# tensorlayer/TLXCV

Hardware: AMD Instinct MI355X
Metric: images/sec fwd (higher is better)
Workload: dtype f16; 1 GPU; ResNet-50 fp16 forward, 224x224, batch 256 per GPU (BASELINE configs[1]); global_batch=256, per_gpu_batch=256, weights=seeded random (tlxcv_amd.seeded, seed 1), parallelism=single GPU, launch=hipGraph replay of the forward

## Files before the change

include/tlxmi.h:

```cpp
#ifndef TLXMI_H
#define TLXMI_H

#include <stddef.h>
#include <stdint.h>

#ifdef __cplusplus
extern "C" {
#endif

#define TLXMI_VERSION 101

typedef enum tlxmi_status {
    TLXMI_OK = 0,
    TLXMI_ERR_BAD_ARG = -1,
    TLXMI_ERR_UNSUPPORTED = -2,
    TLXMI_ERR_ALIGNMENT = -3,
    TLXMI_ERR_LAUNCH = -4,
    TLXMI_ERR_NO_DEVICE = -5
} tlxmi_status;

typedef enum tlxmi_dtype { TLXMI_F16 = 0, TLXMI_F32 = 1 } tlxmi_dtype;

typedef enum tlxmi_act {
    TLXMI_ACT_NONE = 0,
// ... 89 lines not shown
typedef struct tlxmi_seam_desc {
    int32_t dtype;
    int64_t rows;
    int32_t K1, N1, N2;
    int32_t t2_ld, skip_ld, y_ld, t1_ld;
    int32_t act;
} tlxmi_seam_desc;
int tlxmi_bottleneck_seam_supported(int dtype, int K1, int N1, int N2);
int tlxmi_bottleneck_seam_proj(const tlxmi_seam_desc* d, const void* t2, const void* w3_packed, const float* scale3,
                               const float* shift3, const void* x, const void* wd_packed, const float* scale_d,
                               const float* shift_d, void* y, const void* w1_packed, const float* scale1,
                               const float* shift1, void* t1, void* stream);
int tlxmi_bottleneck_seam(const tlxmi_seam_desc* d, const void* t2, const void* w3_packed, const float* scale3,
                          const float* shift3, const void* skip, void* y, const void* w1_packed, const float* scale1,
                          const float* shift1, void* t1, void* stream);

int tlxmi_group_conv_chunks(int Cin, int Cout, int groups, int dtype);
size_t tlxmi_packed_group_filter_bytes(int Cout, int Cin, int R, int S, int groups, int dtype);
int tlxmi_pack_group_filter(const float* src_oihw, void* dst, int Cout, int Cin, int R, int S, int groups,
                            int dtype, void* stream);
int tlxmi_group_conv2d(const tlxmi_conv2d_desc* d, int groups, const void* x, const void* w_packed,
                       const float* scale, const float* shift, const void* res, void* y, void* stream);
int tlxmi_group_conv2d_small_supported(const tlxmi_conv2d_desc* d, int groups);

int tlxmi_linear_splitk(int dtype, int64_t rows, int K, int Cout, int x_ld, const void* x, const void* w_packed,
                        int splits, void* partials, const float* scale, const float* shift, const void* res,
                        int res_ld, int act, float act_param, uint32_t flags, void* y, int y_ld, void* stream);

int tlxmi_conv2d_splitk_supported(const tlxmi_conv2d_desc* d, int splits);
int tlxmi_conv2d_splitk(const tlxmi_conv2d_desc* d, int splits, const void* x, const void* w_packed, void* partials,
// ... 176 lines not shown
```

tlxcv_amd/_lib.py:

```python
import ctypes as C
import os

_HERE = os.path.dirname(os.path.abspath(__file__))
LIB_PATH = os.path.join(_HERE, "libtlxmi.so")

F16, F32 = 0, 1
ACT_NONE, ACT_RELU, ACT_RELU6, ACT_LEAKY, ACT_HARDSWISH, ACT_HARDSIGMOID, ACT_GELU, ACT_SIGMOID, ACT_SILU = range(9)
EPI_RES_AFTER_ACT = 1
EPI_MAXPOOL_3S2P1 = 4
PLAN_SHARED_HALF = 0x100
PLAN_SHARED_FULL = 0x200
LAYOUT_NHWC, LAYOUT_NCHW = 0, 1


class ConvDesc(C.Structure):
    _fields_ = [(n, C.c_int32) for n in (
        "dtype", "N", "H", "W", "C", "Cout", "R", "S", "stride_h", "stride_w", "pad_h", "pad_w",
        "dil_h", "dil_w", "Ho", "Wo", "x_ld", "y_ld", "res_ld", "y_nstride", "res_nstride", "act")] + [
        ("act_param", C.c_float), ("flags", C.c_uint32)]


class DwConvDesc(C.Structure):
    _fields_ = [(n, C.c_int32) for n in (
        "dtype", "N", "H", "W", "C", "R", "S", "stride_h", "stride_w", "pad_h", "pad_w", "dil_h",
# ... 29 lines not shown
        ("scale", C.c_float), ("mask_mode", C.c_int32)] + [(n, C.c_int64) for n in (
            "q_batch_stride", "q_row_stride", "k_batch_stride", "k_row_stride", "v_batch_stride", "v_row_stride",
            "out_batch_stride", "out_row_stride")]


class CswinAttnDesc(C.Structure):
    _fields_ = [(n, C.c_int32) for n in ("dtype", "B", "H", "W", "hd")] + [("scale", C.c_float)] + [
        (n, C.c_int32) for n in ("branches", "heads")] + [("hs", C.c_int32 * 2), ("ws", C.c_int32 * 2)] + [(n, C.c_int64) for n in (
            "q_batch_stride", "q_row_stride", "k_batch_stride", "k_row_stride", "v_batch_stride", "v_row_stride",
            "out_batch_stride", "out_row_stride")]


class SeamDesc(C.Structure):
    _fields_ = [("dtype", C.c_int32), ("rows", C.c_int64)] + [(n, C.c_int32) for n in (
        "K1", "N1", "N2", "t2_ld", "skip_ld", "y_ld", "t1_ld", "act")]


class PreprocDesc(C.Structure):
    _fields_ = [(n, C.c_int32) for n in ("N", "H", "W", "C", "out_h", "out_w", "kh", "kw", "out_dtype", "layout", "fold_b",
                                         "cpad", "normalize")]


_vp, _i, _f, _u, _l = C.c_void_p, C.c_int, C.c_float, C.c_uint32, C.c_int64

PROTOTYPES = {
    "tlxmi_nchw_to_nhwc": [_vp, _i, _vp, _i, _i, _i, _i, _i, _i, _vp],
    "tlxmi_nchw_to_nhwc_s2d": [_vp, _i, _vp, _i, _i, _i, _i, _i, _i, _i, _vp],
    "tlxmi_patchify": [_vp, _i, _vp, _i, _i, _i, _i, _i, _i, _i, _vp],
    "tlxmi_patch_embed4": [_vp, _i, _vp, _vp, _vp, _vp, _vp, _i, _i, _i, _i, _f, _vp],
    "tlxmi_patch_embed4_pos": [_vp, _i, _vp, _vp, _vp, _vp, _vp, _vp, _i, _i, _i, _i, _f, _vp],
    "tlxmi_nhwc_to_nchw": [_vp, _i, _i, _vp, _i, _i, _i, _i, _i, _vp],
    "tlxmi_pack_filter": [_vp, _vp, _i, _i, _i, _i, _i, _vp],
    "tlxmi_fold_bn": [_vp, _vp, _vp, _vp, _vp, _f, _i, _vp, _vp, _vp],
    "tlxmi_conv2d": [C.POINTER(ConvDesc), _vp, _vp, _vp, _vp, _vp, _vp, _vp],
    "tlxmi_conv2d_splitk": [C.POINTER(ConvDesc), _i, _vp, _vp, _vp, _vp, _vp, _vp, _vp, _vp],
    "tlxmi_bottleneck_seam": [C.POINTER(SeamDesc), _vp, _vp, _vp, _vp, _vp, _vp, _vp, _vp, _vp, _vp, _vp],
    "tlxmi_bottleneck_seam_proj": [C.POINTER(SeamDesc), _vp, _vp, _vp, _vp, _vp, _vp, _vp, _vp, _vp, _vp, _vp, _vp, _vp, _vp],
    "tlxmi_preprocess_u8": [C.POINTER(PreprocDesc), _vp, _vp, _vp, _vp, _vp, _vp, _vp, _vp, _vp, _vp],
    "tlxmi_preprocess_linear_u8": [C.POINTER(PreprocDesc), _vp, _vp, _vp, _vp, _vp, _vp, _vp, _vp, _vp],
    "tlxmi_yolo_iou_aware": [_vp, _vp, _i, _l, _i, _i, _f, _vp],
    "tlxmi_yolo_box": [_vp, _i, _i, _i, _i, _i, _i, _i, _vp, _vp, _f, _i, _i, _f, _vp, _vp, _i, _i, _vp],
    "tlxmi_multiclass_nms": [_vp, _vp, _i, _i, _i, _f, _f, _i, _vp, _vp, _vp, _vp],
    "tlxmi_multiclass_nms_index": [_vp, _vp, _i, _i, _i, _f, _f, _i, _vp, _vp, _vp, _vp, _vp],
    "tlxmi_linear_splitk": [_i, _l, _i, _i, _i, _vp, _vp, _i, _vp, _vp, _vp, _vp, _i, _i, _f, _u, _vp, _i, _vp],
    "tlxmi_group_conv2d": [C.POINTER(ConvDesc), _i, _vp, _vp, _vp, _vp, _vp, _vp, _vp],
    "tlxmi_pack_group_filter": [_vp, _vp, _i, _i, _i, _i, _i, _i, _vp],
    "tlxmi_dwconv2d": [C.POINTER(DwConvDesc), _vp, _vp, _vp, _vp, _vp, _vp],
    "tlxmi_maxpool2d": [_vp, _vp, _i, _i, _i, _i, _i, _i, _i, _i, _i, _i, _i, _i, _i, _i, _i, _vp],
    "tlxmi_avgpool2d": [_vp, _vp, _i, _i, _i, _i, _i, _i, _i, _i, _i, _i, _i, _i, _i, _i, _i, _vp],
    "tlxmi_radix_gap": [_vp, _vp, _i, _i, _i, _i, _i, _i, _i, _vp],
    "tlxmi_split_attention": [_vp, _vp, _vp, _vp, _i, _i, _i, _i, _i, _i, _i, _i, _i, _vp],
    "tlxmi_global_avgpool": [_vp, _vp, _i, _i, _i, _i, _i, _i, _vp],
# ... 30 lines not shown
    "tlxmi_mul": [_vp, _vp, _vp, _i, _l, _i, _i, _i, _i, _vp],
}
_SPECIAL = {
    "tlxmi_version": ([], C.c_int),
    "tlxmi_last_error": ([], C.c_char_p),
    "tlxmi_device_count": ([], C.c_int),
    "tlxmi_packed_filter_bytes": ([_i, _i, _i, _i, _i], C.c_size_t),
    "tlxmi_packed_group_filter_bytes": ([_i, _i, _i, _i, _i, _i], C.c_size_t),
    "tlxmi_group_conv_chunks": ([_i, _i, _i, _i], C.c_int),
    "tlxmi_group_conv2d_small_supported": ([C.POINTER(ConvDesc), _i], C.c_int),
    "tlxmi_conv2d_maxpool_supported": ([C.POINTER(ConvDesc)], C.c_int),
    "tlxmi_conv2d_splitk_supported": ([C.POINTER(ConvDesc), _i], C.c_int),
    "tlxmi_preprocess_u8_workspace_bytes": ([C.POINTER(PreprocDesc)], C.c_size_t),
    "tlxmi_multiclass_nms_workspace_bytes": ([_i, _i], C.c_size_t),
    "tlxmi_bottleneck_seam_supported": ([_i, _i, _i, _i], C.c_int),
    "tlxmi_linear_ln_supported": ([_i, _l, _i, _i, _i, _i], C.c_int),
    "tlxmi_mlp_seam_supported": ([_i, _i, _i, _i], C.c_int),
    "tlxmi_sepconv2d_supported": ([C.POINTER(SepConvDesc)], C.c_int),
    "tlxmi_dwconv7_stats_supported": ([C.POINTER(DwConv7Desc)], C.c_int),
    "tlxmi_preact_conv1x1_supported": ([_i, _l, _i, _i, _i, _i, _i, _i], C.c_int),
    "tlxmi_sr_attention_supported": ([C.POINTER(MhaDesc)], C.c_int),
    "tlxmi_cswin_attention_supported": ([C.POINTER(CswinAttnDesc)], C.c_int),
    "tlxmi_lka_dw_supported": ([C.POINTER(LkaDwDesc)], C.c_int),
    "tlxmi_lka_gate_supported": ([C.POINTER(LkaGateDesc)], C.c_int),
}
ALL_SYMBOLS = sorted(list(PROTOTYPES) + list(_SPECIAL))

TUNE_LIB_PATH = os.environ.get("TLXMI_TUNE_LIB") or os.path.join(_HERE, "libtlxmi_tune.so")

_lib = None
# ... 67 lines not shown
```

tlxcv_amd/csrc/conv_igemm.hip:

```cpp
#include "common.h"
#include <stdio.h>
#include "gemm256.h"
#include "conv_halo.h"
#include "group_conv.h"
#include <stdlib.h>
#include <string.h>

namespace tlxmi {

struct ConvArgs {
    const char* x;
    const char* w;
    char* y;
    const float* scale;
    const float* shift;
    const char* res;
    int N, H, W, C, Cout, R, S, sh, sw, ph, pw, dh, dw, Ho, Wo;
    int x_ld, y_ld, res_ld;
    long y_nstride, res_nstride;
    int strided_n;
    int out_f32;
    int pp_slices;
    int act;
    float act_param;
// ... 474 lines not shown
    if (lds > 64 * 1024)
        if (int rc = raise_lds_limit(fn, 160 * 1024, "conv2d")) return rc;
    void* args[] = {&b};
    hipError_t e = hipLaunchKernel(fn, dim3((unsigned)grid, (unsigned)a.nchunk), dim3(WGM * 128), args, lds, st);
    if (e != hipSuccess) return fail(TLXMI_ERR_LAUNCH, "conv2d: HIP launch failed: %s", hipGetErrorString(e));
    return TLXMI_OK;
}

static bool pp_conv_offsets_ok(int W, int R, int S, int ph, int pw, int dh, int dw, int x_ld, int es) {
    const long long px = (long long)x_ld * es;
    const long long lead = ((long long)ph * W + pw) * px;
    const long long reach = ((long long)(R - 1) * dh * W + (long long)(S - 1) * dw + 1) * px;
    return lead < (1ll << 30) && reach < (1ll << 30);
}

template <typename T> static int dispatch(const ConvArgs& a, hipStream_t st, bool allow_stream = true, bool allow_split = true) {
    const bool pool = (a.flags & TLXMI_EPI_MAXPOOL_3S2P1) != 0;
    if constexpr (sizeof(T) == 2) {
        const int PB = a.C * 2;
        if (pool) {
            if (!(a.nchunk == 1 && !a.overhang && a.sh == 1 && a.sw == 1 && a.dh == 1 && a.dw == 1 && conv_halo_pool_ok(a.R, a.S, PB, a.Ho, a.Wo) &&
                  conv_halo_pool_act_ok(a.act) && !a.strided_n && a.vec_io && !a.res && a.Cout % 8 == 0 && a.Cout <= 128 && a.y_bytes != 0))
                return fail(TLXMI_ERR_UNSUPPORTED, "conv2d: TLXMI_EPI_MAXPOOL_3S2P1 needs the fp16 4x4 / 16-channel stem geometry (Wo = 112, even Ho, no residual)");
            HaloArgs h;
            h.x = a.x; h.w = a.w; h.y = a.y; h.scale = a.scale; h.shift = a.shift; h.res = nullptr;
            h.N = a.N; h.H = a.H; h.W = a.W; h.Cout = a.Cout; h.R = a.R; h.S = a.S; h.ph = a.ph; h.pw = a.pw;
            h.Ho = a.Ho; h.Wo = a.Wo; h.HoWo = a.HoWo; h.x_ld = a.x_ld; h.y_ld = a.y_ld; h.res_ld = 0;
            h.PB = PB; h.Kp_bytes = a.Kp_bytes; h.act = a.act; h.act_param = a.act_param; h.flags = a.flags;
            h.tpi = a.Ho / 2;
            h.ntn = (a.Cout + 63) / 64; h.nt = 0;
// ... 30 lines not shown
            h.x_bytes = a.x_bytes; h.w_bytes = a.w_bytes; h.y_bytes = a.y_bytes;
            h.res_bytes = a.res ? (unsigned)((long long)a.M * a.res_ld * 2) : 0u;
            if ((long)h.nring * h.PWp * PB + 512 <= 160 * 1024) {
                trace_launched("halo", a.M, a.Cout);
                return launch_conv_halo(h, st, num_cus());
            }
        }
    }
    if (pool) return fail(TLXMI_ERR_UNSUPPORTED, "conv2d: TLXMI_EPI_MAXPOOL_3S2P1 is an fp16-only fusion");
    struct Cand { int bm, bn; float eff; };
    const double flops = 2.0 * a.M * (double)a.Cout * a.kchunks * (16 / (int)sizeof(T));
    const double obytes = (double)a.M * a.Cout * sizeof(T) * (a.res ? 2.0 : 1.0);
    const double obi = obytes / flops;
    constexpr int NC = 12;
    Cand cands[NC] = {{128, 128, 1.00f}, {64, 128, 0.85f}, {128, 64, 0.85f}, {64, 64, 0.70f}, {256, 128, 0.90f},
                      {256, 256, 1.12f}, {256, 128, 1.20f}, {256, 256, 1.40f}, {256, 256, 1.50f}, {128, 256, 1.25f},
                      {256, 128, 1.25f}, {256, 256, 0.f}};
    const bool gemm128_ok = a.nchunk == 1 && a.R == 1 && a.S == 1 && a.ph == 0 && a.pw == 0 && a.sh == 1 && a.sw == 1 && !a.strided_n &&
                            a.vec_io && a.Cout % 8 == 0 && a.y_bytes != 0 && a.Cout >= 128 && a.ktiles >= 2 &&
                            (!a.res || (long long)a.M * a.res_ld * (long long)sizeof(T) < (1ll << 31));
    const bool gemm256_ok = gemm128_ok && a.Cout >= 256;
    const int tpk = a.cpt / 8;
    const bool strided1x1 = a.R == 1 && a.S == 1 && a.ph == 0 && a.pw == 0 && (a.sh > 1 || a.sw > 1);
    const bool as_conv = !(a.R == 1 && a.S == 1 && a.ph == 0 && a.pw == 0 && a.sh == 1 && a.sw == 1);
    const bool dilated = a.dh != 1 || a.dw != 1;
    const bool pp_dil_ok = !dilated || (tune_int("TLXMI_PP_DIL", 1) != 0 && pp_conv_offsets_ok(a.W, a.R, a.S, a.ph, a.pw, a.dh, a.dw, a.x_ld, (int)sizeof(T)));
    const bool pp_conv128_ok = a.nchunk == 1 && !a.overhang && ((a.S == 3 && a.R <= 3) || strided1x1) && pp_dil_ok && !a.strided_n &&
                               a.vec_io && a.Cout % 8 == 0 && a.Cout >= 128 && a.y_bytes != 0 && a.cpt % 8 == 0 && (tpk & (tpk - 1)) == 0 &&
                               (!a.res || (long long)a.M * a.res_ld * (long long)sizeof(T) < (1ll << 31));
    const bool pp_conv_ok = pp_conv128_ok && a.Cout >= 256;
    const long wreg = tune_int("TLXMI_WREG", 1);
// ... 572 lines not shown
    d.x_ld = x_ld; d.y_ld = Cout; d.act = TLXMI_ACT_NONE;
    const int rc = conv2d_impl(&d, splits, x, w_packed, nullptr, nullptr, nullptr, partials, stream, false, true, pstride * 4);
    if (rc != TLXMI_OK) return rc;
    const long total = (long)rows * Cout;
    const unsigned grid = (unsigned)((total + 255) / 256 < 8192 ? (total + 255) / 256 : 8192);
    if (dtype == TLXMI_F16)
        hipLaunchKernelGGL((splitk_reduce_kernel<half_t>), dim3(grid), dim3(256), 0, as_stream(stream), (const float*)partials, splits, (long)rows, Cout,
                           (long)pstride, scale, shift, (const half_t*)res, res_ld, act, act_param, flags, (half_t*)y, y_ld);
    else
        hipLaunchKernelGGL((splitk_reduce_kernel<float>), dim3(grid), dim3(256), 0, as_stream(stream), (const float*)partials, splits, (long)rows, Cout,
                           (long)pstride, scale, shift, (const float*)res, res_ld, act, act_param, flags, (float*)y, y_ld);
    return check_launch("linear_splitk");
}

namespace tlxmi {
static inline int cin_pad(int Cin, int dtype) { const int v = 16 / (int)elt_size(dtype); return (Cin + v - 1) / v * v; }
static inline int kpad_elems(int Cin, int R, int S, int dtype);
static int kpad_elems_of(int Cin, int R, int S, int dtype) { return kpad_elems(Cin, R, S, dtype); }
static inline int kpad_elems(int Cin, int R, int S, int dtype) {
    const int es = (int)elt_size(dtype);
    const int kbytes = R * S * cin_pad(Cin, dtype) * es;
    return ((kbytes + 127) / 128 * 128) / es;
}
template <typename T>
__global__ void pack_filter_kernel(const float* __restrict__ src, T* __restrict__ dst, int Cout, int Cin, int R,
                                   int S, int Cinp, int Kp, long total) {
    for (long i = (long)blockIdx.x * blockDim.x + threadIdx.x; i < total; i += (long)gridDim.x * blockDim.x) {
        const int k = (int)(i % Kp);
        const int o = (int)(i / Kp);
        const int c = k % Cinp, tap = k / Cinp;
// ... 68 lines not shown
```

tlxcv_amd/csrc/gemm256.h:

```cpp
#pragma once
#include <hip/hip_runtime.h>

namespace tlxmi {

struct Gemm256Args {
    const char* x;
    const char* w;
    char* y;
    const float* scale;
    const float* shift;
    const char* res;
    const float* rowstats = nullptr;
    float* stats_out = nullptr;
    int ln_planes = 0;
    float ln_inv_c = 0.f, ln_eps = 0.f;
    int M, Cout, x_ld, y_ld, res_ld;
    int kchunks;
    int ksteps;
    int Kp_bytes;
    int act;
    float act_param;
    unsigned flags;
    int mtiles, ntiles;
    int tiles_full = 0, tiles_total = 0, m_full = 0;
    int gn;
    unsigned x_bytes, w_bytes, y_bytes, res_bytes;
    int debug;
    int conv;
    int cH, cW, cWo, cHoWo, csh, csw, cph, cpw;
    int ctshift, ctaps;
    int kslices = 1, kt_slice = 0;
    long long slice_bytes = 0;
    int cdh = 1, cdw = 1;
};

int launch_gemm256(int dtype, int variant, const Gemm256Args& a, hipStream_t st);
int launch_gemm_pp(int dtype, const Gemm256Args& a, hipStream_t st);
int launch_gemm_pp128(int dtype, const Gemm256Args& a, hipStream_t st);
int launch_gemm_pp_n128(int dtype, const Gemm256Args& a, hipStream_t st);
bool gemm_stream_ok(int dtype, const Gemm256Args& a);
int launch_gemm_stream(int dtype, const Gemm256Args& a, hipStream_t st, int cus);

bool gemm_w4_ok(int dtype, const Gemm256Args& a);
int launch_gemm_w4(int dtype, const Gemm256Args& a, hipStream_t st, int cus);

bool gemm_wreg_ok(int dtype, const Gemm256Args& a);
int launch_gemm_wreg(const Gemm256Args& a, hipStream_t st);

}
```

tlxcv_amd/csrc/gemm_pp.hip:

```cpp
#include "common.h"
#include "gemm256.h"
#include <stdlib.h>

namespace tlxmi {

typedef __attribute__((address_space(3))) void* lds_ptr_pp_t;
static __device__ __forceinline__ void pp_dma16(__amdgpu_buffer_rsrc_t rsrc, char* lds, int voff) {
    __builtin_amdgcn_raw_ptr_buffer_load_lds(rsrc, (lds_ptr_pp_t)lds, 16, voff, 0, 0, 0);
}
static __device__ __forceinline__ __amdgpu_buffer_rsrc_t pp_srd(const char* p, unsigned bytes) {
    return __builtin_amdgcn_make_buffer_rsrc(const_cast<char*>(p), 0, bytes, 0x00020000);
}
static __device__ __forceinline__ u32x4 pp_load16(__amdgpu_buffer_rsrc_t rsrc, int voff) {
    return __builtin_amdgcn_raw_buffer_load_b128(rsrc, voff, 0, 0);
}
static __device__ __forceinline__ void pp_store16_nt(__amdgpu_buffer_rsrc_t rsrc, u32x4 v, int voff) {
    __builtin_amdgcn_raw_buffer_store_b128(v, rsrc, voff, 0, 2);
}
static __device__ __forceinline__ void pp_store16_wb(__amdgpu_buffer_rsrc_t rsrc, u32x4 v, int voff) {
    __builtin_amdgcn_raw_buffer_store_b128(v, rsrc, voff, 0, 0);
}

template <typename T> struct MmaPP;
template <> struct MmaPP<half_t> {
    static __device__ __forceinline__ f32x4 run(u32x4 a, u32x4 b, f32x4 c) {
        return __builtin_amdgcn_mfma_f32_16x16x32_f16(__builtin_bit_cast(half8v, a), __builtin_bit_cast(half8v, b), c, 0, 0, 0);
    }
};
template <> struct MmaPP<float> {
    static __device__ __forceinline__ f32x4 run(u32x4 a, u32x4 b, f32x4 c) {
        f32x4 af = __builtin_bit_cast(f32x4, a), bf = __builtin_bit_cast(f32x4, b);
#pragma unroll
        for (int j = 0; j < 4; ++j) c = __builtin_amdgcn_mfma_f32_16x16x4f32(af[j], bf[j], c, 0, 0, 0);
        return c;
    }
};

template <typename T, int HM, int HN, bool CONV, bool LNF = false, bool DIL = false>
__global__ __launch_bounds__(512) void gemm_pp_kernel(const Gemm256Args a) {
    static_assert(HM + HN >= 3 && HM <= 2 && HN <= 2, "tile is 256x256, 128x256 or 256x128");
    constexpr int ES = (int)sizeof(T);
    constexpr int BM = 128 * HM, BN = 128 * HN;
    constexpr int HALF = 128 * 128;
    constexpr int RX0 = 0, RX1 = HALF, RW0 = HM * HALF, RW1 = (HM + 1) * HALF;
    constexpr int KTB = (HM + HN) * HALF;
    constexpr int NBUF = (HM + HN == 4) ? 2 : 3;
    constexpr int OOB = (int)0x80000000;
    extern __shared__ __attribute__((aligned(16))) char smem[];

    const int t = threadIdx.x, lane = t & 63;
    const int wid = __builtin_amdgcn_readfirstlane(t >> 6);
    const int wr = wid >> 2, wc = wid & 3;

    int tile_m, tile_n;
    {
        const int nb = a.mtiles * a.ntiles, id = a.kslices > 1 ? (int)blockIdx.x % nb : (int)blockIdx.x;
        const int xcd = id & 7, qd = nb >> 3, rm = nb & 7;
        const int L = (xcd < rm ? xcd * (qd + 1) : rm * (qd + 1) + (xcd - rm) * qd) + (id >> 3);
        const int per = a.mtiles * a.gn, p = L / per, r = L - p * per;
        const int gh = a.ntiles - p * a.gn < a.gn ? a.ntiles - p * a.gn : a.gn;
        tile_m = r / gh;
        tile_n = p * a.gn + r - tile_m * gh;
    }
    const int bm0 = tile_m * BM, bn0 = tile_n * BN;
    const int slice = a.kslices > 1 ? (int)blockIdx.x / (a.mtiles * a.ntiles) : 0;
    const int kt0 = slice * a.kt_slice;
    const int ks = a.kslices > 1 ? (a.ksteps - kt0 < a.kt_slice ? a.ksteps - kt0 : a.kt_slice) : a.ksteps;
    const __amdgpu_buffer_rsrc_t xsrd = pp_srd(a.x, a.x_bytes), wsrd = pp_srd(a.w, a.w_bytes);

    const int lrow = lane >> 3;
    const int lc = (lane & 7) ^ ((4 * (wid & 1) + (lane >> 4)) & 7);
    int xo[2][2], wo[2][2];
    unsigned tapmask[2][2];
#pragma unroll
    for (int h = 0; h < 2; ++h)
#pragma unroll
        for (int j = 0; j < 2; ++j) {
            const int m = bm0 + 128 * h + 8 * (wid + 8 * j) + lrow;
            if constexpr (CONV) {
                const bool live = h < HM && m < a.M;
                const int mm = live ? m : 0;
                const int n = mm / a.cHoWo, rem = mm - n * a.cHoWo;
                const int ho = rem / a.cWo, wo_ = rem - ho * a.cWo;
                const int hi0 = ho * a.csh - a.cph, wi0 = wo_ * a.csw - a.cpw;
                xo[h][j] = ((n * a.cH + hi0) * a.cW + wi0) * a.x_ld * ES;
                const int dh = DIL ? a.cdh : 1, dw = DIL ? a.cdw : 1;
                unsigned mk = 0;
#pragma unroll
                for (int tp = 0; tp < 9; ++tp) {
                    const int r = tp / 3, s_ = tp - 3 * r;
                    if (live && tp < a.ctaps && (unsigned)(hi0 + r * dh) < (unsigned)a.cH && (unsigned)(wi0 + s_ * dw) < (unsigned)a.cW) mk |= 1u << tp;
                }
                tapmask[h][j] = mk;
            } else {
                xo[h][j] = (h < HM && m < a.M) ? m * a.x_ld * ES : OOB;
                tapmask[h][j] = 0;
            }
            const int rho = 128 * h + 8 * (wid + 8 * j) + lrow;
            const int n = (rho & ~31) | (((rho >> 2) & 3) << 3) | (((rho >> 4) & 1) << 2) | (rho & 3);
            wo[h][j] = (bn0 + n) * a.Kp_bytes;
        }
    char* const lbase = smem + wid * 1024;
    auto stage_x = [&](int h, int kt, int buf) {
        char* b = lbase + buf * KTB + (h ? RX1 : RX0);
        const bool mine = kt < ks;
        kt += kt0;
        if constexpr (CONV) {
            const int tap = kt >> a.ctshift;
            const int r = (tap * 11) >> 5, s_ = tap - 3 * r;
            const int d = (DIL ? r * a.cdh * a.cW + s_ * a.cdw : r * a.cW + s_) * a.x_ld * ES + (((kt - (tap << a.ctshift)) * 8 + lc) << 4);
#pragma unroll
            for (int j = 0; j < 2; ++j) pp_dma16(xsrd, b + j * 8192, (mine && ((tapmask[h][j] >> tap) & 1u)) ? xo[h][j] + d : OOB);
        } else {
            const int q = kt * 8 + lc;
            const bool in = mine && q < a.kchunks;
#pragma unroll
            for (int j = 0; j < 2; ++j) pp_dma16(xsrd, b + j * 8192, in ? xo[h][j] + q * 16 : OOB);
        }
    };
    auto stage_w = [&](int g, int kt, int buf) {
        const int q = (kt + kt0) * 8 + lc;
        char* b = lbase + buf * KTB + (g ? RW1 : RW0);
        const bool in = kt < ks && q * 16 < a.Kp_bytes;
#pragma unroll
        for (int j = 0; j < 2; ++j) pp_dma16(wsrd, b + j * 8192, in ? wo[g][j] + q * 16 : OOB);
    };

// ... 322 lines not shown
                    for (int h = 0; h < HM; ++h) {
                        const f32x2* q = scr + (h * 2 + wr) * 4 * 64 + lane;
                        const f32x2 p0 = q[0], p1 = q[64], p2 = q[128], p3 = q[192];
                        const int m = bm0 + 128 * h + 64 * wr + lane;
                        if (m < a.M)
                            *reinterpret_cast<f32x2*>(a.stats_out + 2 * ((size_t)m * 4 + (bn0 >> 8))) =
                                f32x2{(p0[0] + p1[0]) + (p2[0] + p3[0]), (p0[1] + p1[1]) + (p2[1] + p3[1])};
                    }
                }
            }
        }
    };
    TLXMI_DISPATCH_ACT(a.act, epi)
}

template <typename T, int HM, int HN, bool CONV, bool LNF = false, bool DIL = false> static int launch_pp_t(const Gemm256Args& a0, hipStream_t st) {
    Gemm256Args a = a0;
    a.debug = (int)tune_int("TLXMI_DEBUG", 0);
    a.mtiles = (a.M + 128 * HM - 1) / (128 * HM);
    a.ntiles = (a.Cout + 128 * HN - 1) / (128 * HN);
    a.gn = a.ntiles;
    if (const long g = tune_int("TLXMI_GS_PANEL", 3); !CONV && g > 0 && g < a.ntiles) a.gn = (int)g;
    const size_t lds = (size_t)(HM + HN == 4 ? 8 : 9) * 128 * 128 + 2 * 256 * sizeof(float);
    const void* fn = reinterpret_cast<const void*>(&gemm_pp_kernel<T, HM, HN, CONV, LNF, DIL>);
    if (int rc = raise_lds_limit(fn, (int)lds, "gemm_pp")) return rc;
    void* args[] = {&a};
    hipError_t e = hipLaunchKernel(fn, dim3((unsigned)(a.mtiles * a.ntiles * (a.kslices > 1 ? a.kslices : 1))), dim3(512), args, lds, st);
    if (e != hipSuccess) return fail(TLXMI_ERR_LAUNCH, "gemm_pp: HIP launch failed: %s", hipGetErrorString(e));
    return TLXMI_OK;
}

template <int HM, int HN> static int launch_pp_conv(int dtype, const Gemm256Args& a, hipStream_t st) {
    if (a.cdh != 1 || a.cdw != 1) {
        if (dtype == TLXMI_F16) return launch_pp_t<half_t, HM, HN, true, false, true>(a, st);
        return launch_pp_t<float, HM, HN, true, false, true>(a, st);
    }
    if (dtype == TLXMI_F16) return launch_pp_t<half_t, HM, HN, true>(a, st);
    return launch_pp_t<float, HM, HN, true>(a, st);
}
// ... 12 lines not shown
    if (a.conv) return launch_pp_conv<1, 2>(dtype, a, st);
    if (a.rowstats || a.stats_out) {
        if (dtype != TLXMI_F16 || (a.Cout & 31) || a.kslices > 1) return fail(TLXMI_ERR_UNSUPPORTED, "gemm_pp: the LayerNorm fold is fp16, Cout %% 32 == 0");
        return launch_pp_t<half_t, 1, 2, false, true>(a, st);
    }
    if (dtype == TLXMI_F16) return launch_pp_t<half_t, 1, 2, false>(a, st);
    return launch_pp_t<float, 1, 2, false>(a, st);
}

int launch_gemm_pp_n128(int dtype, const Gemm256Args& a, hipStream_t st) {
    if (a.conv) return launch_pp_conv<2, 1>(dtype, a, st);
    if (dtype == TLXMI_F16) return launch_pp_t<half_t, 2, 1, false>(a, st);
    return launch_pp_t<float, 2, 1, false>(a, st);
}

}
```

tlxcv_amd/engine.py:

```python
import ctypes as C
import threading

import torch

from . import _lib
from ._lib import (ACT_GELU, ACT_HARDSIGMOID, ACT_HARDSWISH, ACT_LEAKY, ACT_NONE, ACT_RELU, ACT_RELU6,
                   ACT_SIGMOID, ACT_SILU, EPI_RES_AFTER_ACT, F16, F32)

EPI_RES_BCAST_N = 2

_precision = torch.float16

_options = {"splitk": True,
            "attn_comb": True,
            "seams": True,
            "seam256": True,
            "two_streams": True,
            "conv_splitk": True,
            "patch_linear": True,
            "patch_embed4": True,
            "mlp_seam": True,
            "lnfold": True,
            "lnfold_min_rows": 2048,
            "lnfold_min_rows_one_stream": 12000,
            "lnfold_min_c": 256,
            "sepconv": True,
            "dwconv7": True,
            "preact": True,
            "sr_attn": True,
            "lka": True,
            "cswin_attn": True,
# ... 559 lines not shown
        args = (C.byref(d), _p(t2), _p(pk3.buf), _p(scale3), _p(shift3), _p(skip), _p(pkd.buf), _p(sd), _p(hd), _p(y), _p(pk1.buf), _p(scale1),
                _p(shift1), _p(t1), _stream())
    if _probe is None:
        _lib.call(name, *args)
        return y, t1
    es = t2.element_size()
    skip_ch = pk3.Cout if proj is None else proj[0].Cin
    alg_bytes = (rows * (pk3.Cin + skip_ch + pk3.Cout + pk1.Cout) + pk3.Cout * pk3.Cin + pk1.Cout * pk1.Cin) * es
    flops = 2 * rows * (pk3.Cout * pk3.Cin + pk1.Cout * pk1.Cin + (0 if proj is None else pk3.Cout * proj[0].Cin))
    e0, e1 = torch.cuda.Event(enable_timing=True), torch.cuda.Event(enable_timing=True)
    e0.record()
    _lib.call(name, *args)
    e1.record()
    _probe.append((e0, e1, alg_bytes, flops, (N, H, W, pk3.Cin, pk3.Cout, pk1.Cout, "seam" if proj is None else "seam+proj", True)))
    return y, t1


def group_conv2d(x, pk, stride=1, padding=0, dilation=1, scale=None, shift=None, res=None, act=ACT_NONE,
                 act_param=0.0, res_after_act=False):
    need_gpu(x, "input")
    N, H, W, ld = x.shape
    if x.dtype != pk.dtype:
        raise RuntimeError(f"group_conv2d: input dtype {x.dtype} != packed filter dtype {pk.dtype}")
    if ld != pk.Cin:
        raise RuntimeError(f"group_conv2d: input has {ld} channels, filter expects {pk.Cin}")
    sh, sw = _pair(stride)
    ph, pw = _pair(padding)
    dh, dw = _pair(dilation)
    Ho = (H + 2 * ph - dh * (pk.R - 1) - 1) // sh + 1
    Wo = (W + 2 * pw - dw * (pk.S - 1) - 1) // sw + 1
# ... 1015 lines not shown
```

tlxcv_amd/models/classification/resnet.py:

```python
import torch

from ... import engine as E
from ...tlx import nn
from ...tlx import FlattenReshape
from ...tlx.nn import as_nhwc, from_nhwc

__all__ = ['resnet18', 'resnet34', 'resnet50', 'resnet101', 'resnet152', 'wide_resnet50_2', 'wide_resnet101_2',
           'ResNet', 'BasicBlock', 'BottleneckBlock']

_HE = nn.initializers.HeNormal()


def _conv(cin, cout, k, stride=1, padding=0, dilation=1, groups=1, data_format='channels_first'):
    return nn.GroupConv2d(in_channels=cin, out_channels=cout, kernel_size=k, stride=stride, padding=padding,
                          dilation=dilation, n_group=groups, b_init=(), W_init=_HE, data_format=data_format)


class BasicBlock(nn.Module):
    expansion = 1

    def __init__(self, in_channels, out_channels, stride=1, downsample=None, groups=1, base_width=64, dilation=1,
                 batch_norm=None, data_format='channels_first'):
        super().__init__()
        if batch_norm is None:
# ... 10 lines not shown
        self.data_format = data_format

    def forward_nhwc(self, v):
        identity = v
        out = self.conv1.run_nhwc(v, self.bn1, E.ACT_RELU)
        if self.downsample is not None:
            identity = self.downsample[0].run_nhwc(v, self.downsample[1])
        return self.conv2.run_nhwc(out, self.bn2, E.ACT_RELU, res=identity)

    def forward(self, x):
        return from_nhwc(self.forward_nhwc(as_nhwc(x, self.data_format)), self.data_format)


class BottleneckBlock(nn.Module):
    expansion = 4

    def __init__(self, in_channels, out_channels, stride=1, downsample=None, groups=1, base_width=64, dilation=1,
                 batch_norm=None, data_format='channels_first'):
        super().__init__()
        if batch_norm is None:
            batch_norm = nn.BatchNorm2d
        width = int(out_channels * (base_width / 64.0)) * groups
        self.conv1 = _conv(in_channels, width, 1, data_format=data_format)
        self.bn1 = batch_norm(num_features=width, data_format=data_format)
        self.conv2 = _conv(width, width, 3, stride, dilation, dilation, groups, data_format=data_format)
        self.bn2 = batch_norm(num_features=width, data_format=data_format)
        self.conv3 = _conv(width, out_channels * self.expansion, 1, data_format=data_format)
        self.bn3 = batch_norm(num_features=out_channels * self.expansion, data_format=data_format)
        self.relu = nn.ReLU()
        self.downsample = downsample
# ... 9 lines not shown
        return self.conv3.run_nhwc(out, self.bn3, E.ACT_RELU, res=identity)

    def forward(self, x):
        return from_nhwc(self.forward_nhwc(as_nhwc(x, self.data_format)), self.data_format)

    def run_head(self, v, t1=None):
        out = t1 if t1 is not None else self.conv1.run_nhwc(v, self.bn1, E.ACT_RELU)
        return self.conv2.run_nhwc(out, self.bn2, E.ACT_RELU)

    def shortcut(self, v):
        return v if self.downsample is None else self.downsample[0].run_nhwc(v, self.downsample[1])

    def finish(self, out, identity):
        return self.conv3.run_nhwc(out, self.bn3, E.ACT_RELU, res=identity)

    def seam_with(self, nxt, out, v):
        c3, c1 = self.conv3, nxt.conv1
        dt = E.precision()
        if (not E.option("seams") or dt != torch.float16 or c3.n_group != 1 or c1.n_group != 1 or c1.kernel_size != (1, 1) or c1.stride != (1, 1)
                or c1.padding != (0, 0) or c3.biases is not None or c1.biases is not None
                or not E.bottleneck_seam_supported(c3.in_channels, c3.out_channels, c1.out_channels, dt)
                or (c3.in_channels >= 256 and not E.option("seam256"))):
            return None
        n_img = out.shape[0]
        if n_img < 12 or (c3.in_channels >= 256 and (n_img < 96 or n_img > 192)):
            return None
        pk3 = c3._cached("pk", lambda: E.PackedFilter(c3.filters, dt))
        pk1 = c1._cached("pk", lambda: E.PackedFilter(c1.filters, dt))
        s3, h3 = c3._cached(("bn", id(self.bn3)), lambda: self.bn3.folded(None), deps=(self.bn3,))
        s1, h1 = c1._cached(("bn", id(nxt.bn1)), lambda: nxt.bn1.folded(None), deps=(nxt.bn1,))
        if self.downsample is None:
            return E.bottleneck_seam(out, pk3, s3, h3, v, pk1, s1, h1)
        cd, bnd = self.downsample[0], self.downsample[1]
        if (cd.kernel_size == (1, 1) and cd.stride == (1, 1) and cd.padding == (0, 0) and cd.n_group == 1 and cd.biases is None
                and c3.in_channels == 64 and c1.out_channels == 64 and cd.in_channels == 64 and v.shape[-1] == 64):
            pkd = cd._cached("pk", lambda: E.PackedFilter(cd.filters, dt))
            sd, hd = cd._cached(("bn", id(bnd)), lambda: bnd.folded(None), deps=(bnd,))
            return E.bottleneck_seam(out, pk3, s3, h3, v, pk1, s1, h1, proj=(pkd, sd, hd))
        return E.bottleneck_seam(out, pk3, s3, h3, self.shortcut(v), pk1, s1, h1)


def run_bottleneck_chain(blocks, v):
    t1 = None
    for i, blk in enumerate(blocks):
        out = blk.run_head(v, t1)
        t1 = None
        nxt = blocks[i + 1] if i + 1 < len(blocks) else None
        fused = blk.seam_with(nxt, out, v) if isinstance(nxt, BottleneckBlock) else None
        if fused is not None:
            v, t1 = fused
        else:
            v = blk.finish(out, blk.shortcut(v))
    return v


class ResNet(nn.Module):

    def __init__(self, block, depth=50, width=64, num_classes=1000, with_pool=True, groups=1,
                 data_format='channels_first', name=None):
        super().__init__(name=name)
        layer_cfg = {18: [2, 2, 2, 2], 34: [3, 4, 6, 3], 50: [3, 4, 6, 3], 101: [3, 4, 23, 3], 152: [3, 8, 36, 3]}
        layers = layer_cfg[depth]
        self.groups = groups
        self.base_width = width
        self.num_classes = num_classes
        self.with_pool = with_pool
        self.in_channels = 64
        self.dilation = 1
        self.data_format = data_format
        self.conv1 = _conv(3, self.in_channels, 7, 2, 3, data_format=data_format)
        self.bn1 = nn.BatchNorm2d(num_features=self.in_channels, data_format=data_format)
        self.relu = nn.ReLU()
        self.maxpool = nn.MaxPool2d(kernel_size=3, stride=2, padding=1, data_format=data_format)
        self.layer1 = self._make_layer(block, 64, layers[0], data_format=data_format)
        self.layer2 = self._make_layer(block, 128, layers[1], stride=2, data_format=data_format)
        self.layer3 = self._make_layer(block, 256, layers[2], stride=2, data_format=data_format)
        self.layer4 = self._make_layer(block, 512, layers[3], stride=2, data_format=data_format)
        if with_pool:
            self.avgpool = nn.AdaptiveAvgPool2d((1, 1), data_format=data_format)
        self.flatten = FlattenReshape()
        if num_classes > 0:
            self.fc = nn.Linear(in_features=512 * block.expansion, out_features=num_classes)

    def _make_layer(self, block, out_channels, blocks, stride=1, dilate=False, data_format='channels_first'):
        batch_norm = nn.BatchNorm2d
        downsample = None
        previous_dilation = self.dilation
        if dilate:
            self.dilation *= stride
            stride = 1
        if stride != 1 or self.in_channels != out_channels * block.expansion:
            downsample = nn.Sequential([
# ... 68 lines not shown
```

Baseline: 75480 images/sec.

## Fold conv3 and downsample projection into one dual-operand 1x1 GEMM

Adds a dual-operand pipelined GEMM kernel that concatenates conv3's input with a strided gather of the block input along K. This computes the final 1x1 expand conv and the downsample projection, with both BNs folded into one weight and shift, in a single launch with ReLU. It is enabled for the first block of layers 2-4 by default, replacing a separate shortcut conv plus a residual-add epilogue. In exchange, those blocks can no longer use the seam fusion with the next block's conv1, and the strided gather loads of x2 may be less efficient.

```diff
diff --git a/include/tlxmi.h b/include/tlxmi.h
--- a/include/tlxmi.h
+++ b/include/tlxmi.h
@@ -127,6 +127,20 @@
 int tlxmi_bottleneck_seam(const tlxmi_seam_desc* d, const void* t2, const void* w3_packed, const float* scale3,
                           const float* shift3, const void* skip, void* y, const void* w1_packed, const float* scale1,
                           const float* shift1, void* t1, void* stream);
+
+typedef struct tlxmi_proj_desc {
+    int32_t dtype;
+    int32_t N, Ho, Wo;
+    int32_t K1, K2, Cout;
+    int32_t H2, W2, stride;
+    int32_t x_ld, x2_ld, y_ld;
+    int32_t act;
+    float act_param;
+    uint32_t flags;
+} tlxmi_proj_desc;
+int tlxmi_conv1x1_proj_supported(const tlxmi_proj_desc* d, const void* x, const void* x2, const void* w_packed, const void* y);
+int tlxmi_conv1x1_proj(const tlxmi_proj_desc* d, const void* x, const void* x2, const void* w_packed, const float* shift, void* y,
+                       void* stream);
 
 int tlxmi_group_conv_chunks(int Cin, int Cout, int groups, int dtype);
 size_t tlxmi_packed_group_filter_bytes(int Cout, int Cin, int R, int S, int groups, int dtype);
diff --git a/tlxcv_amd/_lib.py b/tlxcv_amd/_lib.py
--- a/tlxcv_amd/_lib.py
+++ b/tlxcv_amd/_lib.py
@@ -67,6 +67,11 @@
 class SeamDesc(C.Structure):
     _fields_ = [("dtype", C.c_int32), ("rows", C.c_int64)] + [(n, C.c_int32) for n in (
         "K1", "N1", "N2", "t2_ld", "skip_ld", "y_ld", "t1_ld", "act")]
+
+
+class ProjDesc(C.Structure):
+    _fields_ = [(n, C.c_int32) for n in ("dtype", "N", "Ho", "Wo", "K1", "K2", "Cout", "H2", "W2", "stride", "x_ld", "x2_ld", "y_ld", "act")] + [
+        ("act_param", C.c_float), ("flags", C.c_uint32)]
 
 
 class PreprocDesc(C.Structure):
@@ -89,6 +94,7 @@
     "tlxmi_conv2d_splitk": [C.POINTER(ConvDesc), _i, _vp, _vp, _vp, _vp, _vp, _vp, _vp, _vp],
     "tlxmi_bottleneck_seam": [C.POINTER(SeamDesc), _vp, _vp, _vp, _vp, _vp, _vp, _vp, _vp, _vp, _vp, _vp],
     "tlxmi_bottleneck_seam_proj": [C.POINTER(SeamDesc), _vp, _vp, _vp, _vp, _vp, _vp, _vp, _vp, _vp, _vp, _vp, _vp, _vp, _vp],
+    "tlxmi_conv1x1_proj": [C.POINTER(ProjDesc), _vp, _vp, _vp, _vp, _vp, _vp],
     "tlxmi_preprocess_u8": [C.POINTER(PreprocDesc), _vp, _vp, _vp, _vp, _vp, _vp, _vp, _vp, _vp, _vp],
     "tlxmi_preprocess_linear_u8": [C.POINTER(PreprocDesc), _vp, _vp, _vp, _vp, _vp, _vp, _vp, _vp, _vp],
     "tlxmi_yolo_iou_aware": [_vp, _vp, _i, _l, _i, _i, _f, _vp],
@@ -149,6 +155,7 @@
     "tlxmi_preprocess_u8_workspace_bytes": ([C.POINTER(PreprocDesc)], C.c_size_t),
     "tlxmi_multiclass_nms_workspace_bytes": ([_i, _i], C.c_size_t),
     "tlxmi_bottleneck_seam_supported": ([_i, _i, _i, _i], C.c_int),
+    "tlxmi_conv1x1_proj_supported": ([C.POINTER(ProjDesc), _vp, _vp, _vp, _vp], C.c_int),
     "tlxmi_linear_ln_supported": ([_i, _l, _i, _i, _i, _i], C.c_int),
     "tlxmi_mlp_seam_supported": ([_i, _i, _i, _i], C.c_int),
     "tlxmi_sepconv2d_supported": ([C.POINTER(SepConvDesc)], C.c_int),
diff --git a/tlxcv_amd/csrc/conv_igemm.hip b/tlxcv_amd/csrc/conv_igemm.hip
--- a/tlxcv_amd/csrc/conv_igemm.hip
+++ b/tlxcv_amd/csrc/conv_igemm.hip
@@ -512,6 +512,8 @@
     return lead < (1ll << 30) && reach < (1ll << 30);
 }
 
+constexpr float kEffPP256 = 1.40f, kEffPP128 = 1.25f;
+
 template <typename T> static int dispatch(const ConvArgs& a, hipStream_t st, bool allow_stream = true, bool allow_split = true) {
     const bool pool = (a.flags & TLXMI_EPI_MAXPOOL_3S2P1) != 0;
     if constexpr (sizeof(T) == 2) {
@@ -572,7 +574,7 @@
     const double obi = obytes / flops;
     constexpr int NC = 12;
     Cand cands[NC] = {{128, 128, 1.00f}, {64, 128, 0.85f}, {128, 64, 0.85f}, {64, 64, 0.70f}, {256, 128, 0.90f},
-                      {256, 256, 1.12f}, {256, 128, 1.20f}, {256, 256, 1.40f}, {256, 256, 1.50f}, {128, 256, 1.25f},
+                      {256, 256, 1.12f}, {256, 128, 1.20f}, {256, 256, kEffPP256}, {256, 256, 1.50f}, {128, 256, kEffPP128},
                       {256, 128, 1.25f}, {256, 256, 0.f}};
     const bool gemm128_ok = a.nchunk == 1 && a.R == 1 && a.S == 1 && a.ph == 0 && a.pw == 0 && a.sh == 1 && a.sw == 1 && !a.strided_n &&
                             a.vec_io && a.Cout % 8 == 0 && a.y_bytes != 0 && a.Cout >= 128 && a.ktiles >= 2 &&
@@ -1175,6 +1177,75 @@
 }
 
 namespace tlxmi {
+static int proj_check(const tlxmi_proj_desc* d, const void* x, const void* x2, const void* w, const void* y, const char** why) {
+    *why = "null descriptor or buffer";
+    if (!d || !x || !x2 || !w || !y) return TLXMI_ERR_BAD_ARG;
+    *why = "non-positive extent";
+    if (d->N <= 0 || d->Ho <= 0 || d->Wo <= 0 || d->H2 <= 0 || d->W2 <= 0 || d->K1 <= 0 || d->K2 <= 0 || d->Cout <= 0 || d->stride <= 0) return TLXMI_ERR_BAD_ARG;
+    *why = "pitch below the channel count";
+    if (d->x_ld < d->K1 || d->x2_ld < d->K2 || d->y_ld < d->Cout) return TLXMI_ERR_BAD_ARG;
+    *why = "bad dtype or activation";
+    if ((d->dtype != TLXMI_F16 && d->dtype != TLXMI_F32) || d->act < TLXMI_ACT_NONE || d->act > TLXMI_ACT_SILU) return TLXMI_ERR_BAD_ARG;
+    *why = "Ho / Wo are not (H2 - 1) / stride + 1, (W2 - 1) / stride + 1";
+    if (d->Ho != (d->H2 - 1) / d->stride + 1 || d->Wo != (d->W2 - 1) / d->stride + 1) return TLXMI_ERR_BAD_ARG;
+    *why = "pointers and pitches must be multiples of 16 bytes";
+    if (!aligned16(x) || !aligned16(x2) || !aligned16(w) || !aligned16(y) || d->x_ld % 8 || d->x2_ld % 8 || d->y_ld % 8) return TLXMI_ERR_ALIGNMENT;
+    *why = "fp16, stride 1 or 2, K1 and K2 multiples of 64, Cout a multiple of 8";
+    if (d->dtype != TLXMI_F16 || d->stride > 2 || d->K1 % 64 || d->K2 % 64 || d->Cout % 8) return TLXMI_ERR_UNSUPPORTED;
+    const long long big = 1ll << 31;
+    const long long rows = (long long)d->N * d->Ho * d->Wo, pix2 = (long long)d->N * d->H2 * d->W2;
+    const long long xb = rows * d->x_ld * 2, x2b = pix2 * d->x2_ld * 2, yb = rows * d->y_ld * 2;
+    const long long wb = ((long long)d->Cout + 255) / 256 * 256 * ((long long)d->K1 + d->K2) * 2;
+    *why = "a tensor of 2 GiB or more (32-bit buffer offsets)";
+    if (xb >= big || x2b >= big || yb >= big || wb >= big) return TLXMI_ERR_UNSUPPORTED;
+    *why = "y overlaps x or x2";
+    const uintptr_t y0 = (uintptr_t)y, y1 = y0 + (uintptr_t)yb;
+    if ((y0 < (uintptr_t)x + (uintptr_t)xb && (uintptr_t)x < y1) || (y0 < (uintptr_t)x2 + (uintptr_t)x2b && (uintptr_t)x2 < y1)) return TLXMI_ERR_UNSUPPORTED;
+    *why = "";
+    return TLXMI_OK;
+}
+}
+
+extern "C" int tlxmi_conv1x1_proj_supported(const tlxmi_proj_desc* d, const void* x, const void* x2, const void* w_packed, const void* y) {
+    const char* why;
+    return tlxmi::proj_check(d, x, x2, w_packed, y, &why) == TLXMI_OK ? 1 : 0;
+}
+
+extern "C" int tlxmi_conv1x1_proj(const tlxmi_proj_desc* d, const void* x, const void* x2, const void* w_packed, const float* shift, void* y,
+                                  void* stream) {
+    using namespace tlxmi;
+    const char* why;
+    if (const int rc = proj_check(d, x, x2, w_packed, y, &why)) return fail(rc, "conv1x1_proj: %s", why);
+    const long long rows = (long long)d->N * d->Ho * d->Wo;
+    Gemm256Args g;
+    g.debug = 0; g.conv = 0;
+    g.x = (const char*)x; g.w = (const char*)w_packed; g.y = (char*)y; g.scale = nullptr; g.shift = shift; g.res = nullptr;
+    g.M = (int)rows; g.Cout = d->Cout; g.x_ld = d->x_ld; g.y_ld = d->y_ld; g.res_ld = 0;
+    g.k1_tiles = d->K1 / 64; g.k2_tiles = d->K2 / 64;
+    g.ksteps = g.k1_tiles + g.k2_tiles; g.kchunks = g.ksteps * 8; g.Kp_bytes = g.ksteps * 128;
+    g.act = d->act; g.act_param = d->act_param; g.flags = d->flags & (TLXMI_PLAN_SHARED_HALF | TLXMI_PLAN_SHARED_FULL);
+    g.mtiles = g.ntiles = 0; g.gn = 1;
+    g.x_bytes = (unsigned)(rows * d->x_ld * 2);
+    g.y_bytes = (unsigned)(((rows - 1) * d->y_ld + d->Cout) * 2);
+    g.res_bytes = 0;
+    g.w_bytes = (unsigned)(((size_t)(d->Cout + 127) / 128 * 128) * (size_t)g.Kp_bytes);
+    g.x2 = (const char*)x2; g.x2_ld = d->x2_ld;
+    g.x2_bytes = (unsigned)((long long)d->N * d->H2 * d->W2 * d->x2_ld * 2);
+    g.dH2 = d->H2; g.dW2 = d->W2; g.dWo = d->Wo; g.dHoWo = d->Ho * d->Wo; g.ds = d->stride;
+    const int cus = (d->flags & TLXMI_PLAN_SHARED_HALF) ? (num_cus() / 2 > 0 ? num_cus() / 2 : 1) : num_cus();
+    const long nt = (d->Cout + 255) / 256;
+    auto price = [&](int bm, float eff) {
+        const long mt = (long)((rows + bm - 1) / bm), blocks = mt * nt, rounds = (blocks + cus - 1) / cus;
+        return (float)blocks / (float)(rounds * cus) * ((float)rows / (float)(mt * bm)) * eff;
+    };
+    const long forced = tune_int("TLXMI_PROJ_TILE", 0);
+    const bool half_height = forced == 1 ? false : forced == 2 ? true : price(128, kEffPP128) > price(256, kEffPP256);
+    trace_launched(half_height ? "pp_dual128" : "pp_dual256", g.M, g.Cout);
+    if (int rc = launch_gemm_pp_dual(g, half_height, as_stream(stream))) return rc;
+    return check_launch("conv1x1_proj");
+}
+
+namespace tlxmi {
 static inline int cin_pad(int Cin, int dtype) { const int v = 16 / (int)elt_size(dtype); return (Cin + v - 1) / v * v; }
 static inline int kpad_elems(int Cin, int R, int S, int dtype);
 static int kpad_elems_of(int Cin, int R, int S, int dtype) { return kpad_elems(Cin, R, S, dtype); }
diff --git a/tlxcv_amd/csrc/gemm256.h b/tlxcv_amd/csrc/gemm256.h
--- a/tlxcv_amd/csrc/gemm256.h
+++ b/tlxcv_amd/csrc/gemm256.h
@@ -32,12 +32,17 @@
     int kslices = 1, kt_slice = 0;
     long long slice_bytes = 0;
     int cdh = 1, cdw = 1;
+    const char* x2 = nullptr;
+    unsigned x2_bytes = 0;
+    int x2_ld = 0, k1_tiles = 0, k2_tiles = 0;
+    int dH2 = 1, dW2 = 1, dWo = 1, dHoWo = 1, ds = 1;
 };
 
 int launch_gemm256(int dtype, int variant, const Gemm256Args& a, hipStream_t st);
 int launch_gemm_pp(int dtype, const Gemm256Args& a, hipStream_t st);
 int launch_gemm_pp128(int dtype, const Gemm256Args& a, hipStream_t st);
 int launch_gemm_pp_n128(int dtype, const Gemm256Args& a, hipStream_t st);
+int launch_gemm_pp_dual(const Gemm256Args& a, bool half_height, hipStream_t st);
 bool gemm_stream_ok(int dtype, const Gemm256Args& a);
 int launch_gemm_stream(int dtype, const Gemm256Args& a, hipStream_t st, int cus);
 
diff --git a/tlxcv_amd/csrc/gemm_pp.hip b/tlxcv_amd/csrc/gemm_pp.hip
--- a/tlxcv_amd/csrc/gemm_pp.hip
+++ b/tlxcv_amd/csrc/gemm_pp.hip
@@ -36,9 +36,10 @@
     }
 };
 
-template <typename T, int HM, int HN, bool CONV, bool LNF = false, bool DIL = false>
+template <typename T, int HM, int HN, bool CONV, bool LNF = false, bool DIL = false, bool DUAL = false>
 __global__ __launch_bounds__(512) void gemm_pp_kernel(const Gemm256Args a) {
     static_assert(HM + HN >= 3 && HM <= 2 && HN <= 2, "tile is 256x256, 128x256 or 256x128");
+    static_assert(!DUAL || (!CONV && !LNF && !DIL && sizeof(T) == 2), "DUAL: fp16 GEMM rows plus one gathered operand");
     constexpr int ES = (int)sizeof(T);
     constexpr int BM = 128 * HM, BN = 128 * HN;
     constexpr int HALF = 128 * 128;
@@ -67,10 +68,12 @@
     const int kt0 = slice * a.kt_slice;
     const int ks = a.kslices > 1 ? (a.ksteps - kt0 < a.kt_slice ? a.ksteps - kt0 : a.kt_slice) : a.ksteps;
     const __amdgpu_buffer_rsrc_t xsrd = pp_srd(a.x, a.x_bytes), wsrd = pp_srd(a.w, a.w_bytes);
+    const __amdgpu_buffer_rsrc_t x2srd = DUAL ? pp_srd(a.x2, a.x2_bytes) : xsrd;
 
     const int lrow = lane >> 3;
     const int lc = (lane & 7) ^ ((4 * (wid & 1) + (lane >> 4)) & 7);
     int xo[2][2], wo[2][2];
+    int xo2[2][2];
     unsigned tapmask[2][2];
 #pragma unroll
     for (int h = 0; h < 2; ++h)
@@ -96,6 +99,13 @@
                 xo[h][j] = (h < HM && m < a.M) ? m * a.x_ld * ES : OOB;
                 tapmask[h][j] = 0;
             }
+            if constexpr (DUAL) {
+                const bool live = h < HM && m < a.M;
+                const int mm = live ? m : 0;
+                const int n = mm / a.dHoWo, rem = mm - n * a.dHoWo;
+                const int ho = rem / a.dWo, wo_ = rem - ho * a.dWo;
+                xo2[h][j] = live ? ((n * a.dH2 + ho * a.ds) * a.dW2 + wo_ * a.ds) * a.x2_ld * ES : OOB;
+            }
             const int rho = 128 * h + 8 * (wid + 8 * j) + lrow;
             const int n = (rho & ~31) | (((rho >> 2) & 3) << 3) | (((rho >> 4) & 1) << 2) | (rho & 3);
             wo[h][j] = (bn0 + n) * a.Kp_bytes;
@@ -111,6 +121,17 @@
             const int d = (DIL ? r * a.cdh * a.cW + s_ * a.cdw : r * a.cW + s_) * a.x_ld * ES + (((kt - (tap << a.ctshift)) * 8 + lc) << 4);
 #pragma unroll
             for (int j = 0; j < 2; ++j) pp_dma16(xsrd, b + j * 8192, (mine && ((tapmask[h][j] >> tap) & 1u)) ? xo[h][j] + d : OOB);
+        } else if constexpr (DUAL) {
+            if (kt < a.k1_tiles) {
+                const int q = kt * 8 + lc;
+#pragma unroll
+                for (int j = 0; j < 2; ++j) pp_dma16(xsrd, b + j * 8192, mine ? xo[h][j] + q * 16 : OOB);
+            } else {
+                const int q = (kt - a.k1_tiles) * 8 + lc;
+                const bool in = mine && kt < a.k1_tiles + a.k2_tiles;
+#pragma unroll
+                for (int j = 0; j < 2; ++j) pp_dma16(x2srd, b + j * 8192, in ? xo2[h][j] + q * 16 : OOB);
+            }
         } else {
             const int q = kt * 8 + lc;
             const bool in = mine && q < a.kchunks;
@@ -463,7 +484,7 @@
     TLXMI_DISPATCH_ACT(a.act, epi)
 }
 
-template <typename T, int HM, int HN, bool CONV, bool LNF = false, bool DIL = false> static int launch_pp_t(const Gemm256Args& a0, hipStream_t st) {
+template <typename T, int HM, int HN, bool CONV, bool LNF = false, bool DIL = false, bool DUAL = false> static int launch_pp_t(const Gemm256Args& a0, hipStream_t st) {
     Gemm256Args a = a0;
     a.debug = (int)tune_int("TLXMI_DEBUG", 0);
     a.mtiles = (a.M + 128 * HM - 1) / (128 * HM);
@@ -471,7 +492,7 @@
     a.gn = a.ntiles;
     if (const long g = tune_int("TLXMI_GS_PANEL", 3); !CONV && g > 0 && g < a.ntiles) a.gn = (int)g;
     const size_t lds = (size_t)(HM + HN == 4 ? 8 : 9) * 128 * 128 + 2 * 256 * sizeof(float);
-    const void* fn = reinterpret_cast<const void*>(&gemm_pp_kernel<T, HM, HN, CONV, LNF, DIL>);
+    const void* fn = reinterpret_cast<const void*>(&gemm_pp_kernel<T, HM, HN, CONV, LNF, DIL, DUAL>);
     if (int rc = raise_lds_limit(fn, (int)lds, "gemm_pp")) return rc;
     void* args[] = {&a};
     hipError_t e = hipLaunchKernel(fn, dim3((unsigned)(a.mtiles * a.ntiles * (a.kslices > 1 ? a.kslices : 1))), dim3(512), args, lds, st);
@@ -514,4 +535,10 @@
     return launch_pp_t<float, 2, 1, false>(a, st);
 }
 
-}
+int launch_gemm_pp_dual(const Gemm256Args& a, bool half_height, hipStream_t st) {
+    if (a.conv || a.kslices > 1 || a.rowstats || a.stats_out || !a.x2 || a.k1_tiles < 1 || a.k2_tiles < 1 || a.ksteps != a.k1_tiles + a.k2_tiles)
+        return fail(TLXMI_ERR_UNSUPPORTED, "gemm_pp: the two-operand form takes plain rows plus one gathered operand (no split K, no LayerNorm fold)");
+    return half_height ? launch_pp_t<half_t, 1, 2, false, false, false, true>(a, st) : launch_pp_t<half_t, 2, 2, false, false, false, true>(a, st);
+}
+
+}
diff --git a/tlxcv_amd/engine.py b/tlxcv_amd/engine.py
--- a/tlxcv_amd/engine.py
+++ b/tlxcv_amd/engine.py
@@ -15,6 +15,7 @@
             "attn_comb": True,
             "seams": True,
             "seam256": True,
+            "proj_fold": 7,
             "two_streams": True,
             "conv_splitk": True,
             "patch_linear": True,
@@ -604,6 +605,52 @@
     e1.record()
     _probe.append((e0, e1, alg_bytes, flops, (N, H, W, pk3.Cin, pk3.Cout, pk1.Cout, "seam" if proj is None else "seam+proj", True)))
     return y, t1
+
+
+def _proj_desc(t2, x2, pk, stride, out_ld, act, act_param, k2):
+    N, Ho, Wo, ld = t2.shape
+    k2 = x2.shape[-1] if k2 is None else int(k2)
+    return _lib.ProjDesc(dtype=dt_code(t2.dtype), N=N, Ho=Ho, Wo=Wo, K1=pk.Cin - k2, K2=k2, Cout=pk.Cout, H2=x2.shape[1],
+                         W2=x2.shape[2], stride=int(stride), x_ld=ld, x2_ld=x2.shape[-1], y_ld=out_ld, act=act, act_param=float(act_param),
+                         flags=plan_flags())
+
+
+def conv1x1_proj_supported(t2, x2, pk, stride, out=None, k2=None):
+    if (t2.dim() != 4 or x2.dim() != 4 or t2.dtype != pk.dtype or x2.dtype != pk.dtype or pk.R != 1 or pk.S != 1 or t2.shape[0] != x2.shape[0]
+            or pk.Cin <= (x2.shape[-1] if k2 is None else k2) or not t2.is_contiguous() or not x2.is_contiguous() or t2.dtype not in (torch.float16, torch.float32)):
+        return False
+    N, Ho, Wo, _ = t2.shape
+    d = _proj_desc(t2, x2, pk, stride, pk.Cout if out is None else out.shape[-1], ACT_NONE, 0.0, k2)
+    y = C.c_void_p(16) if out is None else _p(out)
+    return bool(_lib.load().tlxmi_conv1x1_proj_supported(C.byref(d), _p(t2), _p(x2), _p(pk.buf), y))
+
+
+def conv1x1_proj(t2, x2, pk, stride, shift=None, act=ACT_NONE, act_param=0.0, out=None, k2=None):
+    need_gpu(t2, "input")
+    need_gpu(x2, "shortcut input")
+    if t2.dim() != 4 or x2.dim() != 4 or not t2.is_contiguous() or not x2.is_contiguous() or t2.shape[0] != x2.shape[0]:
+        raise RuntimeError("conv1x1_proj: t2 / x2 must be dense NHWC maps of one batch")
+    if t2.dtype != pk.dtype or x2.dtype != pk.dtype:
+        raise RuntimeError(f"conv1x1_proj: input dtypes {t2.dtype} / {x2.dtype} != packed filter dtype {pk.dtype}")
+    N, Ho, Wo, _ = t2.shape
+    if out is None:
+        out = torch.empty((N, Ho, Wo, pk.Cout), dtype=t2.dtype, device=t2.device)
+    d = _proj_desc(t2, x2, pk, stride, out.shape[-1], act, act_param, k2)
+    M = N * Ho * Wo
+    es = t2.element_size()
+    if getattr(_tls, "act_max", None) is not None:
+        _note_act(t2.numel() * es, x2.numel() * es, M * d.y_ld * es)
+    args = (C.byref(d), _p(t2), _p(x2), _p(pk.buf), _p(shift), _p(out), _stream())
+    if _probe is None:
+        _lib.call("tlxmi_conv1x1_proj", *args)
+        return out
+    alg_bytes = (M * (d.K1 + d.K2) + M * pk.Cout + pk.Cout * pk.Cin) * es
+    flops = 2 * M * pk.Cout * pk.Cin
+    e0, e1 = _probe_pair()
+    _lib.call("tlxmi_conv1x1_proj", *args)
+    e1.record()
+    _probe.append((e0, e1, alg_bytes, flops, (N, Ho, Wo, d.K1, pk.Cout, d.K2, "expand+proj", int(stride))))
+    return out
 
 
 def group_conv2d(x, pk, stride=1, padding=0, dilation=1, scale=None, shift=None, res=None, act=ACT_NONE,
diff --git a/tlxcv_amd/models/classification/resnet.py b/tlxcv_amd/models/classification/resnet.py
--- a/tlxcv_amd/models/classification/resnet.py
+++ b/tlxcv_amd/models/classification/resnet.py
@@ -48,6 +48,7 @@
 
 class BottleneckBlock(nn.Module):
     expansion = 4
+    proj_fold_bit = 7
 
     def __init__(self, in_channels, out_channels, stride=1, downsample=None, groups=1, base_width=64, dilation=1,
                  batch_norm=None, data_format='channels_first'):
@@ -87,6 +88,38 @@
     def finish(self, out, identity):
         return self.conv3.run_nhwc(out, self.bn3, E.ACT_RELU, res=identity)
 
+    def folded_filter(self):
+        c3, cd, bnd = self.conv3, self.downsample[0], self.downsample[1]
+        dt = E.precision()
+
+        def build():
+            s3, h3 = self.bn3.folded(None)
+            sd, hd = bnd.folded(None)
+            w3 = E._f32(c3.filters).reshape(c3.out_channels, c3.in_channels) * s3[:, None]
+            wd = E._f32(cd.filters).reshape(cd.out_channels, cd.in_channels) * sd[:, None]
+            return E.PackedFilter(torch.cat([w3, wd], dim=1), dt), h3 + hd
+        return c3._cached(("projfold", id(cd), id(self.bn3), id(bnd)), build, deps=(cd, self.bn3, bnd))
+
+    def finish_folded(self, out, v):
+        ds = self.downsample
+        if ds is None or E.precision() != torch.float16 or not (E.option_value("proj_fold") & self.proj_fold_bit):
+            return None
+        if len(ds) != 2 or not isinstance(ds[0], nn.GroupConv2d) or not isinstance(ds[1], nn.BatchNorm2d):
+            return None
+        if any(getattr(m, "act", None) is not None for m in (self.bn3, ds[1], self.conv3, ds[0])):
+            return None
+        c3, cd = self.conv3, ds[0]
+        plain = lambda c: (c.kernel_size == (1, 1) and c.padding == (0, 0) and c.dilation == (1, 1) and c.n_group == 1
+                           and c.biases is None and not c.same)
+        if (not plain(c3) or not plain(cd) or c3.stride != (1, 1) or cd.stride not in ((1, 1), (2, 2)) or cd.out_channels != c3.out_channels
+                or c3.in_channels % 64 or cd.in_channels % 64 or c3.out_channels % 8
+                or out.shape[-1] != c3.in_channels or v.shape[-1] != cd.in_channels):
+            return None
+        pk, shift = self.folded_filter()
+        if not E.conv1x1_proj_supported(out, v, pk, cd.stride[0]):
+            return None
+        return E.conv1x1_proj(out, v, pk, cd.stride[0], shift=shift, act=E.ACT_RELU)
+
     def seam_with(self, nxt, out, v):
         c3, c1 = self.conv3, nxt.conv1
         dt = E.precision()
@@ -116,15 +149,19 @@
 def run_bottleneck_chain(blocks, v):
     t1 = None
     for i, blk in enumerate(blocks):
-        out = blk.run_head(v, t1)
-        t1 = None
-        nxt = blocks[i + 1] if i + 1 < len(blocks) else None
-        fused = blk.seam_with(nxt, out, v) if isinstance(nxt, BottleneckBlock) else None
-        if fused is not None:
-            v, t1 = fused
-        else:
-            v = blk.finish(out, blk.shortcut(v))
+        v, t1 = bottleneck_step(blk, blocks[i + 1] if i + 1 < len(blocks) else None, v, t1)
     return v
+
+
+def bottleneck_step(blk, nxt, v, t1=None):
+    out = blk.run_head(v, t1)
+    folded = blk.finish_folded(out, v)
+    if folded is not None:
+        return folded, None
+    fused = blk.seam_with(nxt, out, v) if isinstance(nxt, BottleneckBlock) else None
+    if fused is not None:
+        return fused
+    return blk.finish(out, blk.shortcut(v)), None
 
 
 class ResNet(nn.Module):
@@ -149,6 +186,10 @@
         self.layer2 = self._make_layer(block, 128, layers[1], stride=2, data_format=data_format)
         self.layer3 = self._make_layer(block, 256, layers[2], stride=2, data_format=data_format)
         self.layer4 = self._make_layer(block, 512, layers[3], stride=2, data_format=data_format)
+        if block is BottleneckBlock:
+            self.layer1[0].proj_fold_bit = 0
+            for bit, layer in ((1, self.layer2), (2, self.layer3), (4, self.layer4)):
+                layer[0].proj_fold_bit = bit
         if with_pool:
             self.avgpool = nn.AdaptiveAvgPool2d((1, 1), data_format=data_format)
         self.flatten = FlattenReshape()
```

Measured after the change: 76680 images/sec (median of 6 runs). +1.6%, better.
